# NCAR/SPERR

Measured on AMD Instinct MI355X. Metric: compress+decompress GB/s/GPU on 256^3 fp32 chunks @ BPP=2.0; bitstream-exact vs ref, higher is better.
Workload: dtype f64; 1 GPU; synthetic 1024^3 fp32 turbulence per GPU, 256^3 chunks, BPP=2.0, step = compress + decompress, volume and container resident in HBM; chunks_per_gpu=64, parallelism=chunks farmed over 1 GPU(s), no collective

## Files before the change

sperr_amd/csrc/engine.hip:

```cpp
#include <algorithm>
#include <array>
#include <chrono>
#include <cstdlib>
#include <cstring>
#include <atomic>
#include <deque>
#include <map>
#include <memory>
#include <condition_variable>
#include <mutex>
#include <numeric>
#include <thread>
#include <string>
#include <vector>

#include "../../include/sperr_hip.h"
#include "engine_internal.h"
#include "host_container.hpp"
#include "speck_dec.h"
#include "dequant.h"
#include "speck_enc.h"
#include "speck_tree_host.hpp"
#include "outlier.h"
#include "quality.h"
// ... 365 lines not shown
    return false;
  return lift2_applicable(P.fwd[3].region);
}
constexpr uint32_t kLevel2Floor = 96;
static bool plan_level2(const ShapePlan& P)
{
  const char* env = getenv("SPERR_HIP_XYZ_LEVEL2");
  const int sw = env ? atoi(env) : 1;
  if (sw == 0 || !level2_fits(P))
    return false;
  const uint32_t* r = P.fwd[3].region;
  return sw == 2 || std::min(r[0], std::min(r[1], r[2])) >= kLevel2Floor;
}

static void plan_schedule(ShapePlan& P)
{
  LiftSchedule& S = P.schedule;
  S = LiftSchedule{};
  S.pass.resize(P.fwd.size());
  for (size_t k = 0; k < P.fwd.size(); k++)
    S.pass[k].fuse = pass_fuse_rule(P, k, S.pass[k].inner);
  S.head = fuse_xyz(P) ? LiftSchedule::kHeadXYZ : fuse_xy(P) ? LiftSchedule::kHeadXY : LiftSchedule::kNoHead;
  S.fusable = plan_fusable(P);
  S.brick = S.head == LiftSchedule::kHeadXYZ && S.fusable && P.fwd.size() >= 3;
  for (size_t k = 3; k < P.fwd.size(); k++)
    for (int a = 0; a < 3; a++)
      S.coarseBox[a] = std::max(S.coarseBox[a], P.fwd[k].region[a]);
  S.level2 = plan_level2(P);
}

constexpr int kHiMaxK = 9;
static bool use_lis_hi(const ShapePlan& P, bool tables)
{
  static const bool hiEnv = !(getenv("SPERR_HIP_LIS_HI") && atoi(getenv("SPERR_HIP_LIS_HI")) == 0);
  return hiEnv && tables && P.ht.grids.size() <= 288 && P.ht.roots.size() <= 48 &&
         P.maxK >= 1 && P.maxK <= kHiMaxK;
}
static bool use_tables(const ShapePlan& P)
{
  if (!P.ht.allRegular || P.maxK < 1)
    return false;
  return use_lis_hi(P, true);
}
static bool use_mixed(const ShapePlan& P, bool tables)
{
  static const bool mixEnv = !(getenv("SPERR_HIP_LIS_MIXED") && atoi(getenv("SPERR_HIP_LIS_MIXED")) == 0);
  const bool twoD = (P.ht.flags & spk::kTree2D) != 0;
  if ((!twoD && !mixEnv) || tables || P.ht.cls.empty() || P.ht.roots.size() > 48 || P.ht.grids.size() > 352 ||
      P.ht.mxSlot.size() != P.ht.cls.size())
    return false;
  return 2 * kMxS + 256 <= kMxRing && ((kMxS + kMxM) >> 6) + 5 <= 64 && kMxM >= 192 &&
         mx_smem_bytes(kMxS, kMxM, kMxQ) <= 138u * 1024u;
}
static DecPlanHost plan_list_kernels(const ShapePlan& P, bool tables)
{
  DecPlanHost ph{P.d_initLIS, P.d_initLen, tables, P.l0Level >= 0 && P.ht.grids.size() <= 288,
                 P.l1Level >= 0 && P.ht.grids.size() <= 288, P.maxK};
  ph.l2 = ph.l1 && P.l2Level >= 0;
  ph.hi = use_lis_hi(P, ph.tables);
  ph.mixed = use_mixed(P, tables);
  return ph;
}

int build_plan(ShapePlan& P, size_t dx, size_t dy, size_t dz, bool twoD = false)
{
  const unsigned __int128 samples = (unsigned __int128)dx * dy * dz;
  if (dx == 0 || dy == 0 || dz == 0 || dx > 0xffff || dy > 0xffff || dz > 0xffff || samples > (1ull << 31)) {
    fprintf(stderr, "[sperr_hip] chunk of %zu x %zu x %zu not supported (at most 65535 per axis, 2^31 samples)\n",
            dx, dy, dz);
    return -1;
  }
  P.dims[0] = (uint32_t)dx;
  P.dims[1] = (uint32_t)dy;
  P.dims[2] = (uint32_t)dz;
  P.N = (uint32_t)(dx * dy * dz);
  P.ht = spk::build_tree(dx, dy, dz, twoD, false);
  P.maxK = 0;
  for (const auto& lc : P.ht.levelClass)
    P.maxK = std::max<int>(P.maxK, lc.K);
  const bool tables = use_tables(P);
  if (!tables)
    spk::build_mx_columns(P.ht);
  const spk::HostTree& h = P.ht;
  const uint32_t nlev = h.nlevels;

  std::vector<uint32_t> cap(nlev), levelOff(nlev + 1, 0), initLen(nlev);
  for (uint32_t l = 0; l < nlev; l++) {
    cap[l] = std::max<uint32_t>(h.levelCap[l], (uint32_t)h.initLIS[l].size());
    levelOff[l + 1] = levelOff[l] + cap[l];
    initLen[l] = (uint32_t)h.initLIS[l].size();
  }
  P.lisEntries = levelOff[nlev] + 8;
  std::vector<uint64_t> initLIS(levelOff[nlev] ? levelOff[nlev] : 1, 0);
  for (uint32_t l = 0; l < nlev; l++)
    for (size_t k = 0; k < h.initLIS[l].size(); k++)
      initLIS[levelOff[l] + k] = h.initLIS[l][k];

  std::vector<uint16_t> tileLevel;
  std::vector<uint32_t> tileStart, levelFirstTile(nlev, 0), levelNumTiles(nlev, 0);
  for (uint32_t l = nlev; l-- > 0;) {
    levelFirstTile[l] = (uint32_t)tileLevel.size();
    const uint32_t nt = (cap[l] + kListTile - 1) / kListTile;
    levelNumTiles[l] = nt;
    for (uint32_t t = 0; t < nt; t++) {
      tileLevel.push_back((uint16_t)l);
      tileStart.push_back(t * kListTile);
    }
  }
  P.nListTiles = (uint32_t)tileLevel.size();

  std::vector<uint32_t> depthBlocks;
  P.depthBlockOff.assign(h.maxDepth + 1, 0);
  for (uint32_t d = 0; d < h.maxDepth; d++) {
// ... 4533 lines not shown
```

sperr_amd/csrc/speck_dec.h:

```cpp
#ifndef SPERR_AMD_SPECK_DEC_H
#define SPERR_AMD_SPECK_DEC_H

#include "common.h"

namespace sperrhip {

struct DecState {
  uint32_t active;
  int32_t done;
  uint32_t error;
  int32_t nbp;
  uint32_t cur;
  uint32_t nLip, nRef;
  uint32_t nLeafEv;
  int32_t lastPlane;
  int32_t refPlaneP1;
  uint32_t refPartial;
  uint64_t pos;
  uint64_t avail;
  uint64_t total_bits;
  uint64_t payload;
  uint64_t lipStart, lipBits;
  uint32_t l0Ticket;
  int32_t l0PlaneP1;
// ... 90 lines not shown
  uint32_t queueCap;
  size_t queueStride;
  uint64_t* sigbits;
  size_t sigbitsStride;
  uint32_t treeTabLen;
  uint64_t* leafEv;
  uint32_t leafCap;
  size_t leafStride;
  uint16_t* leafState;
  size_t leafStateStride;
  uint8_t* leafDirty;
  size_t leafDirtyStride;
  const uint32_t* wordLeaf;
  unsigned long long* l0Flags;
  size_t l0FlagStride;
  int32_t l0Level;
  unsigned long long* l0Tab;
  unsigned long long* l1Flags;
  int32_t l1Level;
  unsigned long long* l2Flags;
  int32_t l2Level;
  uint64_t* lisStamps;
  unsigned long long* hiFlags;
  size_t hiFlagStride;
  uint32_t hiW;
  uint32_t hiK;
  uint32_t hiSmemBytes;
  uint32_t hiHop2;
  uint32_t hiGroupsMax;
  uint32_t hiExtra;
  uint32_t hiCand;
  uint32_t hiAhead;
  const uint64_t* iRoots;
  uint32_t iLevels;
  const uint8_t* mxSlot;
  const uint8_t* mxLevelGroup;
  uint32_t mxS, mxM;
  uint32_t mxQ;
  uint32_t mxSmemBytes;
};

struct DecPlanHost {
  const uint64_t* d_initLIS;
  const uint32_t* d_initLen;
  bool tables;
  bool l0;
  bool l1;
  int maxK;
  bool hi = false;
  bool l2 = false;
  bool mixed = false;
  uint32_t gridDiv = 1;
  uint32_t mxGroups = 0;
  bool skipFinish = false;
  uint32_t* d_live = nullptr;
  uint32_t* h_live = nullptr;
  hipEvent_t* liveEv = nullptr;
};
constexpr int kLiveSlots = 24;

constexpr int kTabWMax = 28672;
__host__ __device__ inline uint32_t tab_window(int K, uint32_t smemBytes)
{
  const uint32_t perBit8 = 8u * (uint32_t)(2 * (2 * K - 1) + 4) + 1u;
  const uint32_t fixed = 4 * 8 + 130 * 4 + (uint32_t)(2 * K) * 8 + 64;
  uint32_t w = (uint32_t)(((uint64_t)(smemBytes - fixed) * 8) / perBit8);
  w = w / 1024 * 1024;
  if (w > (uint32_t)kTabWMax)
    w = kTabWMax;
  return w;
}

__host__ __device__ inline uint32_t hi_window(int K, uint32_t smemBytes, uint32_t hop2 = 1)
{
  const uint32_t perBit8 = 8u * (uint32_t)(2 * (2 * K - 1) + (hop2 ? 8 : 4)) + 1u;
  const uint32_t fixed = 4 * 8 + 2 * 130 * 4 + (uint32_t)(2 * K) * 8 + 64;
  uint32_t w = (uint32_t)(((uint64_t)(smemBytes - fixed) * 8) / perBit8);
  w = w / 256 * 256;
  if (w > (uint32_t)kTabWMax)
    w = kTabWMax;
  return w;
}

constexpr int kMxWordsPerRegion = 8;
constexpr uint32_t kMxS = 2048, kMxM = 768, kMxQ = 1024, kMxRing = 8192;
uint32_t mx_smem_bytes(uint32_t S, uint32_t M, uint32_t Q);
int prepare_lis_mx(const DecBuffers& b);
int launch_lis_mx(hipStream_t stream, const DecBuffers& b, int p, uint32_t groups, bool stamps);

int launch_speck_decode(hipStream_t stream, const DecBuffers& b, const DecPlanHost& plan,
                        const uint8_t* container, const uint64_t* d_chunkOff,
                        const uint64_t* d_chunkLen, bool wide_pass, int maxPlanes);

}
#endif
```

sperr_amd/csrc/speck_dec.hip:

```cpp
#include "speck_dec.h"
#include "dequant.h"
#include "bit_words.h"
#include "lis_chain.h"

namespace sperrhip {

using namespace spk;

#define DEC_ACTIVE_OR_RETURN(s, p)                               \
  if (!(s).active || (s).done || (int)(p) >= (s).nbp)            \
    return;

__device__ __forceinline__ uint64_t get64(const uint64_t* words, uint64_t pos)
{
  const uint64_t lo = words[pos >> 6];
  const int sh = (int)(pos & 63);
  return sh ? (lo >> sh) | (words[(pos >> 6) + 1] << (64 - sh)) : lo;
}

__global__ void k_dec_header(DecBuffers b, const uint8_t* container, const uint64_t* chunkOff,
                             const uint64_t* chunkLen, const uint64_t* initLIS,
                             const uint32_t* initLen, int wide_pass)
{
  const uint32_t c = blockIdx.x * blockDim.x + threadIdx.x;
// ... 27 lines not shown
      s.error = 1;
    return;
  }
  cs.mean = d1;
  cs.q = d2;
  if (len < 17 + 9) {
    s.error = 1;
    return;
  }
  const int nbp = p[17];
  uint64_t total_bits;
  memcpy(&total_bits, p + 18, 8);
  uint64_t avail = (len - 26) * 8;
  if (avail > total_bits)
    avail = total_bits;
  s.nbp = nbp;
  s.avail = avail;
  s.total_bits = total_bits;
  s.payload = chunkOff[c] + 26;
  cs.wide = nbp > 32 ? 1u : 0u;
  cs.nbp = nbp;
  cs.total_bits = total_bits;
  s.active = (nbp > 0 && (int)cs.wide == wide_pass) ? 1u : 0u;
  s.iPart = b.iLevels;
  for (uint32_t l = 0; l < b.tree.nlevels; l++) {
    s.listLen[0][l] = initLen[l];
    s.listLen[1][l] = 0;
    for (uint32_t k = 0; k < initLen[l]; k++)
      b.lis[0][c * b.lisStride + b.levelOff[l] + k] = initLIS[b.levelOff[l] + k];
  }
}

__global__ void __launch_bounds__(kThreads)
k_dec_load_words(DecBuffers b, const uint8_t* container)
{
  const uint32_t c = blockIdx.y;
  const DecState& s = b.st[c];
  if (!s.active)
    return;
  const uint64_t nbytes = (s.avail + 7) / 8;
  const uint64_t w = (uint64_t)blockIdx.x * blockDim.x + threadIdx.x;
  if (w * 8 >= nbytes)
    return;
  const uint8_t* p = container + s.payload + w * 8;
  uint64_t v = 0;
  const int n = (int)min((uint64_t)8, nbytes - w * 8);
  for (int k = 0; k < n; k++)
    v |= (uint64_t)p[k] << (8 * k);
  b.stream[c * b.streamStride + w] = v;
}

constexpr int kDecTileWords = kThreads;

__device__ __forceinline__ bool leaf_word(const DecBuffers& b, uint32_t c, uint32_t wi,
                                          uint64_t& born, uint64_t& sig, uint64_t& neg, uint32_t tag)
{
  born = sig = neg = 0;
  if (b.wordLeaf == nullptr)
    return false;
  const uint32_t wl = b.wordLeaf[wi];
  if (wl == 0xffffffffu)
    return false;
  if (tag && b.leafDirty[c * b.leafDirtyStride + (wl >> 5)] != (uint8_t)tag)
    return false;
  const uint32_t sel = (wl & 3u) * 2u;
  const uint4* q = reinterpret_cast<const uint4*>(b.leafState + c * b.leafStateStride + (wl & ~31u));
  uint32_t v[16];
  uint32_t any = 0;
#pragma unroll
  for (int k = 0; k < 4; k++) {
    const uint4 t = q[k];
    v[4 * k] = t.x;
    v[4 * k + 1] = t.y;
    v[4 * k + 2] = t.z;
    v[4 * k + 3] = t.w;
    any |= t.x | t.y | t.z | t.w;
  }
  if (!any)
    return false;
  uint32_t bo[2] = {0, 0}, si[2] = {0, 0}, ne[2] = {0, 0};
#pragma unroll
  for (int k = 0; k < 16; k++) {
    const int h = k >> 3, sh = (k & 7) * 4;
    const uint32_t a = v[k] & 0xffffu, d = v[k] >> 16;
    const uint32_t s4 = ((a >> sel) & 3u) | (((d >> sel) & 3u) << 2);
    const uint32_t n4 = ((a >> (8 + sel)) & 3u) | (((d >> (8 + sel)) & 3u) << 2);
    const uint32_t b4 = ((a & 0xffu) ? 3u : 0u) | ((d & 0xffu) ? 12u : 0u);
    si[h] |= s4 << sh;
    ne[h] |= n4 << sh;
    bo[h] |= b4 << sh;
  }
  born = (uint64_t)bo[0] | ((uint64_t)bo[1] << 32);
  sig = (uint64_t)si[0] | ((uint64_t)si[1] << 32);
  neg = (uint64_t)ne[0] | ((uint64_t)ne[1] << 32);
  return true;
}

__global__ void __launch_bounds__(kThreads) k_dec_count(DecBuffers b, int p)
{
  const uint32_t c = blockIdx.y;
  const DecState& s = b.st[c];
  DEC_ACTIVE_OR_RETURN(s, p);
  __shared__ uint32_t sm[kThreads / 64 + 1];
  __shared__ uint32_t sh_need;
  const uint32_t nw = (b.tree.nvals + 63) / 64;
  constexpr uint32_t kAhead = 8;
  for (uint32_t tile0 = blockIdx.x; tile0 < b.nPixTiles; tile0 += gridDim.x * kAhead) {
  uint32_t needMask = 0;
  const bool skipTest = b.tileBorn != nullptr && b.wordLeaf != nullptr;
  if (skipTest) {
    if (threadIdx.x == 0)
      sh_need = 0;
    uint32_t wl[kAhead], tb[kAhead];
#pragma unroll
    for (uint32_t q = 0; q < kAhead; q++) {
      const uint32_t tile = tile0 + q * gridDim.x;
      const uint32_t wi = tile * kDecTileWords + threadIdx.x;
      tb[q] = tile < b.nPixTiles ? (uint32_t)b.tileBorn[c * b.tileStride + tile] : 0u;
      wl[q] = (tile < b.nPixTiles && wi < nw) ? b.wordLeaf[wi] : 0xfffffffeu;
    }
    uint32_t mine = 0;
#pragma unroll
    for (uint32_t q = 0; q < kAhead; q++) {
      const uint32_t tile = tile0 + q * gridDim.x;
      if (tile >= b.nPixTiles)
        continue;
      bool need = tb[q] != 0;
      if (!need && wl[q] != 0xfffffffeu)
        need = wl[q] == 0xffffffffu || b.leafDirty[c * b.leafDirtyStride + (wl[q] >> 5)] == (uint8_t)(p + 2);
      mine |= need ? 1u << q : 0u;
    }
    __syncthreads();
    if (mine)
      atomicOr(&sh_need, mine);
    __syncthreads();
    needMask = sh_need;
  }
  for (uint32_t q = 0; q < kAhead; q++) {
  const uint32_t tile = tile0 + q * gridDim.x;
  if (tile >= b.nPixTiles)
    break;
  const uint32_t wi = tile * kDecTileWords + threadIdx.x;
  if (skipTest && !((needMask >> q) & 1u)) {
    if (threadIdx.x == 0) {
      b.tileLip[c * b.tileStride + tile] = 0;
      b.tileRef[c * b.tileStride + tile] = 0;
    }
    continue;
// ... 11 lines not shown
      if (lb & ~born) {
        born |= lb;
        b.bornM[c * b.maskPixStride + wi] = born;
      }
      if (ln) {
        const uint64_t sg = b.sign[c * b.signStride + wi];
        if (sg & ln)
          b.sign[c * b.signStride + wi] = sg & ~ln;
      }
    }
    if (fresh | (ls & ~sig)) {
      if (b.refPlanes) {
        const uint64_t found = (fresh | ls) & ~sig;
        if (found && (uint32_t)(p + 1) < b.refNPlanes) {
          uint64_t* pw = b.refPlanes + c * b.refPlaneStride + ref_plane_word((uint32_t)(p + 1), wi);
          *pw = sig ? (*pw | found) : found;
          if (!sig)
            b.wordTop[c * b.wordTopStride + wi] = (uint8_t)(p + 2);
        }
      }
      sig |= fresh | ls;
      *so = sig;
    }
    if (fresh)
      *sn = 0;
    const uint64_t lip = born & ~sig;
    v = (uint32_t)__popcll(lip) | ((uint32_t)__popcll(sig) << 16);
    anyBorn = born != 0;
  }
  if (b.tileBorn != nullptr) {
    const int anyB = __syncthreads_or(anyBorn ? 1 : 0);
    if (threadIdx.x == 0 && anyB)
      b.tileBorn[c * b.tileStride + tile] = 1;
  }
  uint32_t r = v;
#pragma unroll
  for (int d = 32; d > 0; d >>= 1)
    r += (uint32_t)__shfl_xor((int)r, d, 64);
  __syncthreads();
  if ((threadIdx.x & 63) == 0)
    sm[threadIdx.x >> 6] = r;
  __syncthreads();
  if (threadIdx.x == 0) {
    uint32_t tot = 0;
    for (int w = 0; w < kThreads / 64; w++)
      tot += sm[w];
    b.tileLip[c * b.tileStride + tile] = tot & 0xffffu;
    b.tileRef[c * b.tileStride + tile] = tot >> 16;
  }
  }
  }
}

__global__ void __launch_bounds__(kThreads) k_dec_scan(DecBuffers b, int p)
{
  const uint32_t c = blockIdx.x;
  DecState& s = b.st[c];
  DEC_ACTIVE_OR_RETURN(s, p);
  __shared__ uint64_t sm[kThreads / 64 + 1];
  uint32_t* tl = b.tileLip + c * b.tileStride;
  uint32_t* tr = b.tileRef + c * b.tileStride;
  uint32_t* ol = b.tileLipOff + c * b.tileStride;
  uint32_t* orr = b.tileRefOff + c * b.tileStride;
  uint64_t carry = 0;
  for (uint32_t base = 0; base < b.nPixTiles; base += kThreads) {
    const uint32_t i = base + threadIdx.x;
    const uint64_t v = i < b.nPixTiles ? ((uint64_t)tl[i] | ((uint64_t)tr[i] << 32)) : 0;
    uint64_t total;
    const uint64_t ex = block_exclusive_scan<uint64_t>(v, sm, &total) + carry;
    if (i < b.nPixTiles) {
      ol[i] = (uint32_t)ex;
      orr[i] = (uint32_t)(ex >> 32);
    }
    carry += total;
  }
  if (threadIdx.x == 0) {
    s.nLip = (uint32_t)carry;
    s.nRef = (uint32_t)(carry >> 32);
    s.lipStart = s.pos;
    s.l0Ticket = 0;
    s.l1Ticket = 0;
    s.l2Ticket = 0;
    s.hiTicket = 0;
    s.hiCompactDone = 0;
    s.bornCount = 0;
    s.leafCount = 0;
    for (int g = 0; g < 8; g++)
      s.hiBornCnt[g] = s.hiLeafCnt[g] = 0;
  }
}

__global__ void __launch_bounds__(kThreads) k_lip_deposit(DecBuffers b, int p)
{
  const uint32_t c = blockIdx.y;
  const DecState& s = b.st[c];
  DEC_ACTIVE_OR_RETURN(s, p);
  if (s.nLip == 0)
    return;
  __shared__ uint32_t sm[kThreads / 64 + 1];
  const uint32_t nw = (b.tree.nvals + 63) / 64;
  const uint64_t* rs = b.lipSig + c * b.lipResStride;
  const uint64_t* rn = b.lipNeg + c * b.lipResStride;
  for (uint32_t tile = blockIdx.x; tile < b.nPixTiles; tile += gridDim.x) {
    if (b.tileLip[c * b.tileStride + tile] == 0)
      continue;
    const uint32_t wi = tile * kDecTileWords + threadIdx.x;
    uint64_t lip = 0;
    if (wi < nw)
      lip = b.bornM[c * b.maskPixStride + wi] & ~b.sigOld[c * b.maskPixStride + wi];
    uint32_t total;
    const uint32_t ex = block_exclusive_scan<uint32_t>((uint32_t)__popcll(lip), sm, &total) +
                        b.tileLipOff[c * b.tileStride + tile];
    const uint32_t n = (uint32_t)__popcll(lip);
    if (n == 0)
      continue;
    const uint32_t sh = ex & 63u;
    uint64_t vs = rs[ex >> 6] >> sh, vn = rn[ex >> 6] >> sh;
    if (sh && sh + n > 64) {
      vs |= rs[(ex >> 6) + 1] << (64 - sh);
      vn |= rn[(ex >> 6) + 1] << (64 - sh);
    }
    if (n < 64) {
      vs &= (1ull << n) - 1;
      vn &= (1ull << n) - 1;
    }
    if (vs == 0)
      continue;
    uint64_t outS = vs, outN = vn;
    spread_under_mask(lip, outS, outN);
    b.sigNew[c * b.maskPixStride + wi] |= outS;
    if (outN)
      b.sign[c * b.signStride + wi] &= ~outN;
  }
}

__device__ __forceinline__ uint64_t lip_word(const uint64_t* words, const DecState& s,
                                             uint64_t w, uint64_t nbits)
{
  const uint64_t pos = s.lipStart + w * 64;
  uint64_t v = get64(words, pos);
  if (pos + 64 > s.avail)
    v = pos >= s.avail ? 0 : (v & ((1ull << (s.avail - pos)) - 1));
// ... 2755 lines not shown
        CT v2 = cv[u];
        if (v2 == 0)
          v2 = initPrev;
        if (p >= 1)
          v2 = sw[u] ? v2 + half : v2 - half;
        else if (sw[u])
          v2 += 1;
        coef[idx[u]] = v2;
      }
    }
    LDS_ONLY_BARRIER();
  }
}

__global__ void __launch_bounds__(kThreads) k_ref_deposit(DecBuffers b, int p)
{
  const uint32_t c = blockIdx.y;
  const DecState& s = b.st[c];
  DEC_ACTIVE_OR_RETURN(s, p);
  if ((uint32_t)p >= b.refNPlanes)
    return;
  __shared__ uint32_t sm[kThreads / 64 + 1];
  const uint32_t nw = (b.tree.nvals + 63) / 64;
  const uint64_t* words = b.stream + c * b.streamStride;
  uint64_t* planes = b.refPlanes + c * b.refPlaneStride;
  const uint64_t avail = s.avail, pos0 = s.pos;
  const bool partial = pos0 + (uint64_t)s.nRef > avail;
  for (uint32_t tile = blockIdx.x; tile < b.nPixTiles; tile += gridDim.x) {
    if (b.tileRef[c * b.tileStride + tile] == 0)
      continue;
    const uint32_t wi = tile * kDecTileWords + threadIdx.x;
    const uint64_t sig = wi < nw ? b.sigOld[c * b.maskPixStride + wi] : 0ull;
    const uint32_t cnt = (uint32_t)__popcll(sig);
    uint32_t total;
    const uint32_t o = block_exclusive_scan_lds<uint32_t>(cnt, sm, &total);
    if (cnt == 0)
      continue;
    const uint64_t at = pos0 + (uint64_t)b.tileRefOff[c * b.tileStride + tile] + o;
    const uint32_t n = at >= avail ? 0u : (uint32_t)min((uint64_t)cnt, avail - at);
    uint64_t res = 0, got = 0;
    if (n) {
      const uint64_t bits = get64(words, at);
      res = n < 64 ? bits & ((1ull << n) - 1) : bits;
      got = n < 64 ? (1ull << n) - 1 : ~0ull;
      if (cnt != 64)
        spread_under_mask(sig, res, got);
    }
    planes[ref_plane_word((uint32_t)p, wi)] = res;
    if (partial)
      b.refMask[c * b.maskPixStride + wi] = got;
  }
}

__global__ void __launch_bounds__(kThreads) k_ref_assemble(DecBuffers b)
{
  const uint32_t c = blockIdx.y;
  const DecState& s = b.st[c];
  const uint32_t nw = (uint32_t)(b.coefStride / 64);
  const uint32_t nwv = (b.tree.nvals + 63) / 64;
  const uint32_t lane = threadIdx.x & 63u;
  uint32_t* coef = reinterpret_cast<uint32_t*>(b.coef) + c * b.coefStride;
  constexpr uint32_t kW = 8;
  const uint32_t wave = (uint32_t)__builtin_amdgcn_readfirstlane((int)((blockIdx.x * kThreads + threadIdx.x) >> 6));
  const uint32_t nwave = (gridDim.x * kThreads) >> 6;
  if (!s.active || s.nbp == 0) {
    for (uint32_t w = wave; w < nw; w += nwave)
      coef[(size_t)w * 64 + lane] = 0;
    return;
  }
  const int lastPlane = s.lastPlane, refPlane = s.refPlaneP1 - 1;
  const bool partial = s.refPartial != 0;
  const int pLow = refPlane >= 0 ? refPlane : lastPlane + 1;
  const int nbp = min(s.nbp, (int)b.refNPlanes);
  const uint64_t* planes = b.refPlanes + c * b.refPlaneStride;
  const uint64_t* sigOld = b.sigOld + c * b.maskPixStride;
  const uint64_t* sigNew = b.sigNew + c * b.maskPixStride;
  const uint64_t* refMask = b.refMask + c * b.maskPixStride;
  const uint8_t* wordTop = b.wordTop + c * b.wordTopStride;
  const int scheme = b.coefSigned != 0 ? coef_scheme(s) : 0;
  const uint64_t* sign = b.sign + c * b.signStride;
  for (uint32_t w0 = wave * kW; w0 + kW <= nw; w0 += nwave * kW) {
    uint64_t so[kW], sn[kW], rm[kW], sg[kW];
    int top[kW], maxTop = 0;
    uint64_t any = 0;
    const uint32_t tops[2] = {reinterpret_cast<const uint32_t*>(wordTop + w0)[0], reinterpret_cast<const uint32_t*>(wordTop + w0)[1]};
#pragma unroll
    for (uint32_t u = 0; u < kW; u++) {
      const uint32_t w = w0 + u;
      const bool in = w < nwv;
      so[u] = sigOld[w];
      sn[u] = sigNew[w];
      rm[u] = refMask[w];
      sg[u] = sign[in ? w : 0u];
      if (!in)
        so[u] = sn[u] = 0;
      top[u] = so[u] ? min((int)((tops[u >> 2] >> (8 * (u & 3))) & 0xffu), nbp) : 0;
      maxTop = max(maxTop, top[u]);
      any |= so[u] | sn[u];
    }
    uint32_t M[kW];
#pragma unroll
    for (uint32_t u = 0; u < kW; u++)
      M[u] = 0;
    if (any && maxTop > pLow) {
      const int nPl = maxTop - pLow;
      const uint32_t myU = lane & 7u, myPs = lane >> 3;
// ... 55 lines not shown
        if (scheme)
          v = coef_scheme_pack(v, ((sg[u] >> lane) & 1ull) != 0, scheme);
      }
      coef[(size_t)w * 64 + lane] = v;
    }
  }
}

__global__ void __launch_bounds__(kThreads) k_dec_fold(DecBuffers b)
{
  const uint32_t c = blockIdx.y;
  const DecState& s = b.st[c];
  if (!s.active || s.nbp == 0)
    return;
  const uint32_t nw = (b.tree.nvals + 63) / 64;
  const uint32_t wi = blockIdx.x * blockDim.x + threadIdx.x;
  if (wi >= nw)
    return;
  uint64_t lb, ls, ln;
  if (!leaf_word(b, c, wi, lb, ls, ln, (uint32_t)s.lastPlane + 1u))
    return;
  const uint64_t fresh = ls & ~b.sigOld[c * b.maskPixStride + wi];
  if (fresh)
    b.sigNew[c * b.maskPixStride + wi] |= fresh;
  if (ln) {
    const uint64_t sg = b.sign[c * b.signStride + wi];
    if (sg & ln)
      b.sign[c * b.signStride + wi] = sg & ~ln;
  }
}

template <typename CT>
__global__ void __launch_bounds__(kThreads) k_dec_finish(DecBuffers b)
{
  const uint32_t c = blockIdx.y;
  const DecState& s = b.st[c];
  if (!s.active || s.nbp == 0)
    return;
  const uint32_t n = b.tree.nvals;
  const uint32_t i = blockIdx.x * blockDim.x + threadIdx.x;
  if (i >= n)
    return;
  const uint64_t m = 1ull << (i & 63);
  const bool isNew = (b.sigNew[c * b.maskPixStride + (i >> 6)] & m) != 0;
  const bool isOld = (b.sigOld[c * b.maskPixStride + (i >> 6)] & m) != 0;
  if (!isNew && !isOld)
    return;
  CT* coef = reinterpret_cast<CT*>(b.coef) + c * b.coefStride;
  if (coef[i] != 0)
    return;
  coef[i] = never_refined<CT>(s.lastPlane + (isNew ? 0 : 1));
}

__global__ void k_dec_plane_end(DecBuffers b, int p)
{
  const uint32_t c = blockIdx.x * blockDim.x + threadIdx.x;
  if (c >= b.nchunks)
    return;
  DecState& s = b.st[c];
  DEC_ACTIVE_OR_RETURN(s, p);
  const uint64_t room = s.avail - s.pos;
  s.refPlaneP1 = p + 1;
  s.refPartial = (uint64_t)s.nRef > room ? 1u : 0u;
  s.pos += min((uint64_t)s.nRef, room);
  if (s.pos >= s.avail || p == 0)
    s.done = 1;
}

__global__ void __launch_bounds__(kThreads) k_dec_live(DecBuffers b, uint32_t* out)
{
  uint32_t live = 0;
  for (uint32_t c = threadIdx.x; c < b.nchunks; c += blockDim.x)
    live += (b.st[c].active && !b.st[c].done) ? 1u : 0u;
  live = (uint32_t)__syncthreads_count(live != 0);
  if (threadIdx.x == 0)
    *out = live;
}

int launch_speck_decode(hipStream_t stream, const DecBuffers& b, const DecPlanHost& plan,
                        const uint8_t* container, const uint64_t* d_chunkOff,
                        const uint64_t* d_chunkLen, bool wide_pass, int maxPlanes)
{
  const uint32_t nc = b.nchunks;
  const dim3 perChunk((nc + 63) / 64);
  LAUNCH_K(k_dec_header, perChunk, dim3(64), 0, stream, b, container, d_chunkOff,
                     d_chunkLen, plan.d_initLIS, plan.d_initLen, wide_pass ? 1 : 0);
  const uint32_t wordBlocks = (uint32_t)((b.streamStride + kThreads - 1) / kThreads);
  LAUNCH_K(k_dec_load_words, dim3(wordBlocks, nc), dim3(kThreads), 0, stream, b,
                     container);
  const uint32_t tokBlocks = (uint32_t)((b.tokStride + kThreads - 1) / kThreads);
  const uint32_t gdiv = std::max<uint32_t>(1u, plan.gridDiv);
  static const uint32_t tileCapEnv = tune_getenv("SPERR_HIP_TILE_GRID") ? (uint32_t)atoi(tune_getenv("SPERR_HIP_TILE_GRID")) : 0u;
  const uint32_t tileCap = tileCapEnv ? tileCapEnv : 1536u;
  const uint32_t tokSegGrid = capped_blocks((uint32_t)(b.tokStride / kLipSeg + 1), nc, kGridCap / gdiv);
  const uint32_t tokGrid = capped_blocks(tokBlocks, nc, kGridCap / gdiv), tileGrid = capped_blocks(b.nPixTiles, nc, tileCap / gdiv);
  static const uint32_t l0Total = tune_getenv("SPERR_HIP_L0_WGS") ? (uint32_t)atoi(tune_getenv("SPERR_HIP_L0_WGS")) : 512u;
  static const uint32_t l01Cap = tune_getenv("SPERR_HIP_L01_CAP") ? (uint32_t)atoi(tune_getenv("SPERR_HIP_L01_CAP")) : 64u;
  const uint32_t l0Groups = std::min<uint32_t>(l01Cap, std::max<uint32_t>(1, l0Total / nc));
  if (plan.tables && plan.l0) {
    if (set_max_dyn_lds(reinterpret_cast<const void*>(&k_lis_l0), (int)kL0Smem) ||
        set_max_dyn_lds(reinterpret_cast<const void*>(&k_lis_l1), (int)kL1Smem) ||
        set_max_dyn_lds(reinterpret_cast<const void*>(&k_lis_l2), (int)kL2Smem))
      return -1;
  }
  static const uint32_t l1Total = tune_getenv("SPERR_HIP_L1_WGS") ? (uint32_t)atoi(tune_getenv("SPERR_HIP_L1_WGS")) : 512u;
  const uint32_t l1Groups = std::min<uint32_t>(l01Cap, std::max<uint32_t>(1, l1Total / nc));
  static const uint32_t l2Total = tune_getenv("SPERR_HIP_L2_WGS") ? (uint32_t)atoi(tune_getenv("SPERR_HIP_L2_WGS")) : 512u;
  const uint32_t l2Groups = std::min<uint32_t>(l01Cap, std::max<uint32_t>(1, l2Total / nc));
  static const uint32_t l2Min = tune_getenv("SPERR_HIP_L2_MIN") ? (uint32_t)std::max(1, atoi(tune_getenv("SPERR_HIP_L2_MIN"))) : 512u;
  const uint32_t placeGrid = capped_blocks((uint32_t)((b.bornStride + kThreads - 1) / kThreads), nc, kGridCap / gdiv);
  static const uint32_t hiTotal = tune_getenv("SPERR_HIP_HI_WGS") ? (uint32_t)atoi(tune_getenv("SPERR_HIP_HI_WGS")) : 128u;
  const uint32_t hiGroups = std::min<uint32_t>(std::max<uint32_t>(1, b.hiGroupsMax), std::max<uint32_t>(1, hiTotal / nc));
  static const uint32_t mxTotal = getenv("SPERR_HIP_MX_WGS") ? (uint32_t)atoi(getenv("SPERR_HIP_MX_WGS")) : 208u;
  const uint32_t mxGroups = std::min<uint32_t>(std::min<uint32_t>(8u, std::max<uint32_t>(1, b.hiGroupsMax)),
                                               plan.mxGroups ? plan.mxGroups : std::max<uint32_t>(1, mxTotal / nc));
  if (plan.mixed && prepare_lis_mx(b))
    return -1;
  if (plan.tables && plan.hi) {
    if (set_max_dyn_lds(reinterpret_cast<const void*>(&k_lis_hi<uint32_t>), (int)b.hiSmemBytes) ||
        set_max_dyn_lds(reinterpret_cast<const void*>(&k_lis_hi<uint64_t>), (int)b.hiSmemBytes))
      return -1;
  }
#define LAUNCH_CT(kern, ...)                    \
  do {                                          \
    if constexpr (sizeof(CT) == 4)              \
      LAUNCH_K(kern<uint32_t>, __VA_ARGS__);    \
    else                                        \
      LAUNCH_K(kern<uint64_t>, __VA_ARGS__);    \
  } while (0)
  auto plane = [&](auto ct, int p) -> int {
    using CT = decltype(ct);
    LAUNCH_K(k_dec_count, dim3(tileGrid, nc), dim3(kThreads), 0, stream, b, p);
    LAUNCH_K(k_dec_scan, dim3(nc), dim3(kThreads), 0, stream, b, p);
    LAUNCH_K(k_lip_words, dim3(tokSegGrid, nc), dim3(kThreads), 0, stream, b, p);
    LAUNCH_K(k_lip_scan, dim3(nc), dim3(kThreads), 0, stream, b, p);
    LAUNCH_CT(k_lip_apply, dim3(tokGrid, nc), dim3(kThreads), 0, stream, b, p);
    LAUNCH_K(k_lip_deposit, dim3(tileGrid, nc), dim3(kThreads), 0, stream, b, p);
    if (plan.tables) {
      if (plan.l0)
        LAUNCH_K(k_lis_l0, dim3(l0Groups, nc), dim3(kL0Threads), kL0Smem, stream, b, p);
      if (plan.l1)
        LAUNCH_K(k_lis_l1, dim3(l1Groups, nc), dim3(kL1Threads), kL1Smem, stream, b, p);
      if (plan.l2)
        LAUNCH_K(k_lis_l2, dim3(l2Groups, nc), dim3(kL2Threads), kL2Smem, stream, b, p, l2Min);
      if (!plan.hi)
        return -1;
      LAUNCH_CT(k_lis_hi, dim3(hiGroups, nc), dim3(kTabThreads), b.hiSmemBytes, stream, b, p);
      LAUNCH_K(k_lis_compact, dim3(b.tree.nlevels, nc), dim3(kTabThreads), 0, stream, b, p);
    }
    else if (plan.mixed) {
      if (launch_lis_mx(stream, b, p, mxGroups, b.lisStamps != nullptr))
        return -1;
      LAUNCH_K(k_lis_compact, dim3(b.tree.nlevels, nc), dim3(kTabThreads), 0, stream, b, p);
    }
    else
      LAUNCH_CT(k_lis_walk, dim3(nc), dim3(64), 0, stream, b, p);
    if (plan.tables || plan.mixed) {
      if (b.nSlots) {
        LAUNCH_K(k_place_scan, dim3(b.nSlots, nc), dim3(kTabThreads), 0, stream, b, p);
        LAUNCH_K(k_place_scatter, dim3(placeGrid, nc), dim3(kThreads), 0, stream, b, p);
      }
      LAUNCH_K(k_leaf_apply, dim3(capped_blocks(1024, nc, kGridCap / gdiv), nc), dim3(kThreads), 0, stream, b, p);
    }
    if (b.refPlanes && sizeof(CT) == 4)
      LAUNCH_K(k_ref_deposit, dim3(tileGrid, nc), dim3(kThreads), 0, stream, b, p);
    else
      LAUNCH_CT(k_ref_apply2, dim3(tileGrid, nc), dim3(kThreads), 0, stream, b, p);
    return 0;
  };
#undef LAUNCH_CT
  for (int p = maxPlanes - 1; p >= 0; p--) {
    if (wide_pass ? plane(uint64_t{}, p) : plane(uint32_t{}, p))
      return -1;
    LAUNCH_K(k_dec_plane_end, perChunk, dim3(64), 0, stream, b, p);
    const int planesDone = maxPlanes - p;
    if (plan.d_live && p > 0 && planesDone >= 16 && planesDone % 2 == 0 && plan.h_live && plan.liveEv) {
      const int k = (planesDone - 16) / 2;
      if (k < kLiveSlots) {
        LAUNCH_K(k_dec_live, dim3(1), dim3(kThreads), 0, stream, b, plan.d_live + k);
        HIP_CHECK(hipMemcpyAsync(plan.h_live + k, plan.d_live + k, sizeof(uint32_t), hipMemcpyDeviceToHost, stream));
        HIP_CHECK(hipEventRecord(plan.liveEv[k], stream));
        if (k >= 1) {
          HIP_CHECK(hipEventSynchronize(plan.liveEv[k - 1]));
          if (plan.h_live[k - 1] == 0)
            break;
        }
      }
    }
  }
  {
    const uint32_t n = b.tree.nvals;
    if ((plan.tables || plan.mixed) && b.wordLeaf)
      LAUNCH_K(k_dec_fold, dim3(((n + 63) / 64 + kThreads - 1) / kThreads, nc), dim3(kThreads), 0,
               stream, b);
    if (b.refPlanes && !wide_pass)
      LAUNCH_K(k_ref_assemble, dim3(capped_blocks((uint32_t)((b.coefStride / 64 + 15) / 16), nc, kGridCapWide), nc),
               dim3(kThreads), 0, stream, b);
    if (!plan.skipFinish) {
      if (wide_pass)
        LAUNCH_K(k_dec_finish<uint64_t>, dim3((n + kThreads - 1) / kThreads, nc), dim3(kThreads), 0,
                 stream, b);
      else
        LAUNCH_K(k_dec_finish<uint32_t>, dim3((n + kThreads - 1) / kThreads, nc), dim3(kThreads), 0,
                 stream, b);
    }
  }
  HIP_CHECK(hipGetLastError());
  return 0;
}

}
```

Measured before the change: 69.84 GB/s.

## Fuse refinement deposit with next plane's pixel count and scan into turn kernels

Adds a k_pix_turn kernel that does the current plane's refinement-bit deposit and the next plane's per-tile count pass in one sweep over the pixel tiles. It prefetches the next word's state and skips tiles that need no work. A k_dec_turn kernel then merges the plane-end bookkeeping with the next plane's scan. Together these replace four kernel launches per bit plane with two, and cut repeated reads of the sig, born and leaf state. The fused path is on by default for large chunks and can be disabled with SPERR_HIP_PIX_TURN=0. It adds complexity to bitstream-exact ordering and register pressure from the prefetch.

```diff
diff --git a/sperr_amd/csrc/engine.hip b/sperr_amd/csrc/engine.hip
--- a/sperr_amd/csrc/engine.hip
+++ b/sperr_amd/csrc/engine.hip
@@ -441,6 +441,17 @@
   return 2 * kMxS + 256 <= kMxRing && ((kMxS + kMxM) >> 6) + 5 <= 64 && kMxM >= 192 &&
          mx_smem_bytes(kMxS, kMxM, kMxQ) <= 138u * 1024u;
 }
+constexpr uint32_t kPixTurnFloor = 64;
+static bool plan_pix_turn(const ShapePlan& P)
+{
+  const char* env = getenv("SPERR_HIP_PIX_TURN");
+  const int sw = env ? atoi(env) : 1;
+  if (sw == 0)
+    return false;
+  const size_t decTiles = (round_up((size_t)P.N, 512) / 64 + kThreads - 1) / kThreads;
+  return sw == 2 || decTiles >= kPixTurnFloor;
+}
+
 static DecPlanHost plan_list_kernels(const ShapePlan& P, bool tables)
 {
   DecPlanHost ph{P.d_initLIS, P.d_initLen, tables, P.l0Level >= 0 && P.ht.grids.size() <= 288,
@@ -448,6 +459,7 @@
   ph.l2 = ph.l1 && P.l2Level >= 0;
   ph.hi = use_lis_hi(P, ph.tables);
   ph.mixed = use_mixed(P, tables);
+  ph.pixTurn = plan_pix_turn(P);
   return ph;
 }
 
diff --git a/sperr_amd/csrc/speck_dec.h b/sperr_amd/csrc/speck_dec.h
--- a/sperr_amd/csrc/speck_dec.h
+++ b/sperr_amd/csrc/speck_dec.h
@@ -166,6 +166,7 @@
   bool mixed = false;
   uint32_t gridDiv = 1;
   uint32_t mxGroups = 0;
+  bool pixTurn = false;
   bool skipFinish = false;
   uint32_t* d_live = nullptr;
   uint32_t* h_live = nullptr;
diff --git a/sperr_amd/csrc/speck_dec.hip b/sperr_amd/csrc/speck_dec.hip
--- a/sperr_amd/csrc/speck_dec.hip
+++ b/sperr_amd/csrc/speck_dec.hip
@@ -103,6 +103,42 @@
 
 constexpr int kDecTileWords = kThreads;
 
+__device__ __forceinline__ bool leaf_states(const DecBuffers& b, uint32_t c, uint32_t wl,
+                                            uint64_t& born, uint64_t& sig, uint64_t& neg)
+{
+  const uint32_t sel = (wl & 3u) * 2u;
+  const uint4* q = reinterpret_cast<const uint4*>(b.leafState + c * b.leafStateStride + (wl & ~31u));
+  uint32_t v[16];
+  uint32_t any = 0;
+#pragma unroll
+  for (int k = 0; k < 4; k++) {
+    const uint4 t = q[k];
+    v[4 * k] = t.x;
+    v[4 * k + 1] = t.y;
+    v[4 * k + 2] = t.z;
+    v[4 * k + 3] = t.w;
+    any |= t.x | t.y | t.z | t.w;
+  }
+  if (!any)
+    return false;
+  uint32_t bo[2] = {0, 0}, si[2] = {0, 0}, ne[2] = {0, 0};
+#pragma unroll
+  for (int k = 0; k < 16; k++) {
+    const int h = k >> 3, sh = (k & 7) * 4;
+    const uint32_t a = v[k] & 0xffffu, d = v[k] >> 16;
+    const uint32_t s4 = ((a >> sel) & 3u) | (((d >> sel) & 3u) << 2);
+    const uint32_t n4 = ((a >> (8 + sel)) & 3u) | (((d >> (8 + sel)) & 3u) << 2);
+    const uint32_t b4 = ((a & 0xffu) ? 3u : 0u) | ((d & 0xffu) ? 12u : 0u);
+    si[h] |= s4 << sh;
+    ne[h] |= n4 << sh;
+    bo[h] |= b4 << sh;
+  }
+  born = (uint64_t)bo[0] | ((uint64_t)bo[1] << 32);
+  sig = (uint64_t)si[0] | ((uint64_t)si[1] << 32);
+  neg = (uint64_t)ne[0] | ((uint64_t)ne[1] << 32);
+  return true;
+}
+
 __device__ __forceinline__ bool leaf_word(const DecBuffers& b, uint32_t c, uint32_t wi,
                                           uint64_t& born, uint64_t& sig, uint64_t& neg, uint32_t tag)
 {
@@ -114,37 +150,7 @@
     return false;
   if (tag && b.leafDirty[c * b.leafDirtyStride + (wl >> 5)] != (uint8_t)tag)
     return false;
-  const uint32_t sel = (wl & 3u) * 2u;
-  const uint4* q = reinterpret_cast<const uint4*>(b.leafState + c * b.leafStateStride + (wl & ~31u));
-  uint32_t v[16];
-  uint32_t any = 0;
-#pragma unroll
-  for (int k = 0; k < 4; k++) {
-    const uint4 t = q[k];
-    v[4 * k] = t.x;
-    v[4 * k + 1] = t.y;
-    v[4 * k + 2] = t.z;
-    v[4 * k + 3] = t.w;
-    any |= t.x | t.y | t.z | t.w;
-  }
-  if (!any)
-    return false;
-  uint32_t bo[2] = {0, 0}, si[2] = {0, 0}, ne[2] = {0, 0};
-#pragma unroll
-  for (int k = 0; k < 16; k++) {
-    const int h = k >> 3, sh = (k & 7) * 4;
-    const uint32_t a = v[k] & 0xffffu, d = v[k] >> 16;
-    const uint32_t s4 = ((a >> sel) & 3u) | (((d >> sel) & 3u) << 2);
-    const uint32_t n4 = ((a >> (8 + sel)) & 3u) | (((d >> (8 + sel)) & 3u) << 2);
-    const uint32_t b4 = ((a & 0xffu) ? 3u : 0u) | ((d & 0xffu) ? 12u : 0u);
-    si[h] |= s4 << sh;
-    ne[h] |= n4 << sh;
-    bo[h] |= b4 << sh;
-  }
-  born = (uint64_t)bo[0] | ((uint64_t)bo[1] << 32);
-  sig = (uint64_t)si[0] | ((uint64_t)si[1] << 32);
-  neg = (uint64_t)ne[0] | ((uint64_t)ne[1] << 32);
-  return true;
+  return leaf_states(b, c, wl, born, sig, neg);
 }
 
 __global__ void __launch_bounds__(kThreads) k_dec_count(DecBuffers b, int p)
@@ -262,12 +268,8 @@
   }
 }
 
-__global__ void __launch_bounds__(kThreads) k_dec_scan(DecBuffers b, int p)
+__device__ __forceinline__ void dec_scan_chunk(const DecBuffers& b, DecState& s, uint32_t c, uint64_t* sm)
 {
-  const uint32_t c = blockIdx.x;
-  DecState& s = b.st[c];
-  DEC_ACTIVE_OR_RETURN(s, p);
-  __shared__ uint64_t sm[kThreads / 64 + 1];
   uint32_t* tl = b.tileLip + c * b.tileStride;
   uint32_t* tr = b.tileRef + c * b.tileStride;
   uint32_t* ol = b.tileLipOff + c * b.tileStride;
@@ -298,6 +300,15 @@
     for (int g = 0; g < 8; g++)
       s.hiBornCnt[g] = s.hiLeafCnt[g] = 0;
   }
+}
+
+__global__ void __launch_bounds__(kThreads) k_dec_scan(DecBuffers b, int p)
+{
+  const uint32_t c = blockIdx.x;
+  DecState& s = b.st[c];
+  DEC_ACTIVE_OR_RETURN(s, p);
+  __shared__ uint64_t sm[kThreads / 64 + 1];
+  dec_scan_chunk(b, s, c, sm);
 }
 
 __global__ void __launch_bounds__(kThreads) k_lip_deposit(DecBuffers b, int p)
@@ -3159,6 +3170,233 @@
   }
 }
 
+struct PixWord {
+  uint64_t sig, fresh, born;
+  uint32_t wl;
+  uint32_t refOff;
+};
+__device__ __forceinline__ PixWord pix_word_load(const DecBuffers& b, uint32_t c, uint32_t tile0, uint32_t todo,
+                                                 uint32_t refTiles, uint32_t countTiles, uint32_t nw)
+{
+  PixWord w{0ull, 0ull, 0ull, 0xffffffffu, 0u};
+  if (todo == 0)
+    return w;
+  const uint32_t q = (uint32_t)__ffs((int)todo) - 1u;
+  const uint32_t tile = tile0 + q * gridDim.x;
+  const uint32_t wi = tile * kDecTileWords + threadIdx.x;
+  if ((refTiles >> q) & 1u)
+    w.refOff = b.tileRefOff[c * b.tileStride + tile];
+  if (wi < nw) {
+    w.sig = b.sigOld[c * b.maskPixStride + wi];
+    if ((countTiles >> q) & 1u) {
+      w.fresh = b.sigNew[c * b.maskPixStride + wi];
+      w.born = b.bornM[c * b.maskPixStride + wi];
+      if (b.wordLeaf != nullptr)
+        w.wl = b.wordLeaf[wi];
+    }
+  }
+  return w;
+}
+
+__global__ void __launch_bounds__(kThreads, 5) k_pix_turn(DecBuffers b, int p)
+{
+  const uint32_t c = blockIdx.y;
+  const DecState& s = b.st[c];
+  if (!s.active || s.done)
+    return;
+  const bool inPlane = p < s.nbp;
+  const uint64_t avail = s.avail, pos0 = s.pos;
+  const uint32_t nRef = s.nRef;
+  const bool refOn = inPlane && (uint32_t)p < b.refNPlanes;
+  const bool endsHere = inPlane && (p == 0 || (uint64_t)nRef >= avail - pos0);
+  const bool countOn = !endsHere && p - 1 >= 0 && p - 1 < s.nbp;
+  if (!refOn && !countOn)
+    return;
+  const bool partial = inPlane && pos0 + (uint64_t)nRef > avail;
+  __shared__ uint32_t smRef[2][kThreads / 64];
+  __shared__ uint32_t smCnt[2][kThreads / 64];
+  __shared__ uint32_t smBorn[2][kThreads / 64];
+  uint32_t refRow = 0, cntRow = 0;
+  __shared__ uint32_t sh_need[2];
+  const uint32_t nw = (b.tree.nvals + 63) / 64;
+  const uint64_t* words = b.stream + c * b.streamStride;
+  constexpr uint32_t kAhead = 8;
+  const bool skipTest = b.tileBorn != nullptr && b.wordLeaf != nullptr;
+  uint32_t round = 0;
+  for (uint32_t tile0 = blockIdx.x; tile0 < b.nPixTiles; tile0 += gridDim.x * kAhead, round ^= 1u) {
+    uint32_t needMask = 0, refMaskT = 0;
+    if (refOn) {
+#pragma unroll
+      for (uint32_t q = 0; q < kAhead; q++) {
+        const uint32_t tile = tile0 + q * gridDim.x;
+        if (tile < b.nPixTiles && b.tileRef[c * b.tileStride + tile] != 0)
+          refMaskT |= 1u << q;
+      }
+    }
+    if (countOn && skipTest) {
+      if (threadIdx.x == 0)
+        sh_need[round] = 0;
+      uint32_t wl[kAhead], tb[kAhead];
+#pragma unroll
+      for (uint32_t q = 0; q < kAhead; q++) {
+        const uint32_t tile = tile0 + q * gridDim.x;
+        const uint32_t wi = tile * kDecTileWords + threadIdx.x;
+        tb[q] = tile < b.nPixTiles ? (uint32_t)b.tileBorn[c * b.tileStride + tile] : 0u;
+        wl[q] = (tile < b.nPixTiles && wi < nw) ? b.wordLeaf[wi] : 0xfffffffeu;
+      }
+      uint32_t mine = 0;
+#pragma unroll
+      for (uint32_t q = 0; q < kAhead; q++) {
+        const uint32_t tile = tile0 + q * gridDim.x;
+        if (tile >= b.nPixTiles)
+          continue;
+        bool need = tb[q] != 0;
+        if (!need && wl[q] != 0xfffffffeu)
+          need = wl[q] == 0xffffffffu || b.leafDirty[c * b.leafDirtyStride + (wl[q] >> 5)] == (uint8_t)(p + 1);
+        mine |= need ? 1u << q : 0u;
+      }
+      __syncthreads();
+      if (mine)
+        atomicOr(&sh_need[round], mine);
+      __syncthreads();
+      needMask = sh_need[round];
+    }
+    else if (countOn)
+      needMask = (1u << kAhead) - 1u;
+    uint32_t todo = 0;
+    for (uint32_t q = 0; q < kAhead; q++) {
+      const uint32_t tile = tile0 + q * gridDim.x;
+      if (tile >= b.nPixTiles)
+        break;
+      if (countOn && !((needMask >> q) & 1u) && threadIdx.x == 0) {
+        b.tileLip[c * b.tileStride + tile] = 0;
+        b.tileRef[c * b.tileStride + tile] = 0;
+      }
+      todo |= (((refMaskT | needMask) >> q) & 1u) << q;
+    }
+    PixWord nx = pix_word_load(b, c, tile0, todo, refMaskT, needMask, nw);
+    uint32_t nxDirty = 0;
+    if (nx.wl != 0xffffffffu)
+      nxDirty = b.leafDirty[c * b.leafDirtyStride + (nx.wl >> 5)];
+    while (todo) {
+      const uint32_t q = (uint32_t)__ffs((int)todo) - 1u;
+      todo &= todo - 1u;
+      const uint32_t tile = tile0 + q * gridDim.x;
+      const uint32_t wi = tile * kDecTileWords + threadIdx.x;
+      const bool doRef = (refMaskT >> q) & 1u, doCount = (needMask >> q) & 1u;
+      const bool in = wi < nw;
+      const PixWord cur = nx;
+      const uint32_t curDirty = nxDirty;
+      nx = pix_word_load(b, c, tile0, todo, refMaskT, needMask, nw);
+      uint64_t sig = cur.sig;
+      uint32_t cnt = 0, n = 0;
+      uint64_t at = 0;
+      if (doRef) {
+        cnt = (uint32_t)__popcll(sig);
+        const uint32_t inc = wave_inclusive_scan(cnt);
+        if ((threadIdx.x & 63u) == 63u)
+          smRef[refRow][threadIdx.x >> 6] = inc;
+        LDS_ONLY_BARRIER();
+        uint32_t base = 0;
+        for (uint32_t w = 0; w < (threadIdx.x >> 6); w++)
+          base += smRef[refRow][w];
+        refRow ^= 1u;
+        at = pos0 + (uint64_t)cur.refOff + base + inc - cnt;
+        n = (cnt == 0 || at >= avail) ? 0u : (uint32_t)min((uint64_t)cnt, avail - at);
+      }
+      const bool hasRef = cnt != 0;
+      uint64_t w0 = 0, w1 = 0;
+      if (n) {
+        w0 = words[at >> 6];
+        w1 = words[(at >> 6) + 1];
+      }
+      if (nx.wl != 0xffffffffu)
+        nxDirty = b.leafDirty[c * b.leafDirtyStride + (nx.wl >> 5)];
+      uint64_t lb = 0, ls = 0, ln = 0;
+      bool leafHit = false;
+      if (cur.wl != 0xffffffffu && curDirty == (uint32_t)(uint8_t)(p + 1) && cur.born != ~0ull)
+        leafHit = leaf_states(b, c, cur.wl, lb, ls, ln);
+      uint64_t res = 0, got = 0;
+      if (n) {
+        const int sh = (int)(at & 63);
+        const uint64_t bits = sh ? (w0 >> sh) | (w1 << (64 - sh)) : w0;
+        res = n < 64 ? bits & ((1ull << n) - 1) : bits;
+        got = n < 64 ? (1ull << n) - 1 : ~0ull;
+        if (cnt != 64)
+          spread_under_mask(sig, res, got);
+      }
+      uint64_t* pw = b.refPlanes + c * b.refPlaneStride + ref_plane_word((uint32_t)p, wi);
+      if (!doCount) {
+        if (hasRef) {
+          *pw = res;
+          if (partial)
+            b.refMask[c * b.maskPixStride + wi] = got;
+        }
+        continue;
+      }
+      uint32_t v = 0;
+      bool anyBorn = false;
+      if (in) {
+        const uint64_t fresh = cur.fresh;
+        uint64_t born = cur.born;
+        if (leafHit) {
+          if (lb & ~born) {
+            born |= lb;
+            b.bornM[c * b.maskPixStride + wi] = born;
+          }
+          if (ln) {
+            const uint64_t sg = b.sign[c * b.signStride + wi];
+            if (sg & ln)
+              b.sign[c * b.signStride + wi] = sg & ~ln;
+          }
+        }
+        uint64_t found = 0;
+        if (fresh | (ls & ~sig)) {
+          found = (fresh | ls) & ~sig;
+          if ((uint32_t)p >= b.refNPlanes)
+            found = 0;
+        }
+        if (hasRef || found) {
+          *pw = res | found;
+          if (!sig)
+            b.wordTop[c * b.wordTopStride + wi] = (uint8_t)(p + 1);
+        }
+        if (fresh | (ls & ~sig)) {
+          sig |= fresh | ls;
+          b.sigOld[c * b.maskPixStride + wi] = sig;
+        }
+        if (fresh)
+          b.sigNew[c * b.maskPixStride + wi] = 0;
+        const uint64_t lip = born & ~sig;
+        v = (uint32_t)__popcll(lip) | ((uint32_t)__popcll(sig) << 16);
+        anyBorn = born != 0;
+      }
+      uint32_t r = v;
+#pragma unroll
+      for (int d = 32; d > 0; d >>= 1)
+        r += (uint32_t)__shfl_xor((int)r, d, 64);
+      const bool waveBorn = __ballot(anyBorn ? 1 : 0) != 0ull;
+      if ((threadIdx.x & 63u) == 0u) {
+        smCnt[cntRow][threadIdx.x >> 6] = r;
+        smBorn[cntRow][threadIdx.x >> 6] = waveBorn ? 1u : 0u;
+      }
+      LDS_ONLY_BARRIER();
+      if (threadIdx.x == 0) {
+        uint32_t tot = 0, anyB = 0;
+        for (int w = 0; w < kThreads / 64; w++) {
+          tot += smCnt[cntRow][w];
+          anyB |= smBorn[cntRow][w];
+        }
+        b.tileLip[c * b.tileStride + tile] = tot & 0xffffu;
+        b.tileRef[c * b.tileStride + tile] = tot >> 16;
+        if (b.tileBorn != nullptr && anyB)
+          b.tileBorn[c * b.tileStride + tile] = 1;
+      }
+      cntRow ^= 1u;
+    }
+  }
+}
+
 __global__ void __launch_bounds__(kThreads) k_ref_assemble(DecBuffers b)
 {
   const uint32_t c = blockIdx.y;
@@ -3320,6 +3558,16 @@
   coef[i] = never_refined<CT>(s.lastPlane + (isNew ? 0 : 1));
 }
 
+__device__ __forceinline__ void dec_plane_end_chunk(DecState& s, int p)
+{
+  const uint64_t room = s.avail - s.pos;
+  s.refPlaneP1 = p + 1;
+  s.refPartial = (uint64_t)s.nRef > room ? 1u : 0u;
+  s.pos += min((uint64_t)s.nRef, room);
+  if (s.pos >= s.avail || p == 0)
+    s.done = 1;
+}
+
 __global__ void k_dec_plane_end(DecBuffers b, int p)
 {
   const uint32_t c = blockIdx.x * blockDim.x + threadIdx.x;
@@ -3327,12 +3575,28 @@
     return;
   DecState& s = b.st[c];
   DEC_ACTIVE_OR_RETURN(s, p);
-  const uint64_t room = s.avail - s.pos;
-  s.refPlaneP1 = p + 1;
-  s.refPartial = (uint64_t)s.nRef > room ? 1u : 0u;
-  s.pos += min((uint64_t)s.nRef, room);
-  if (s.pos >= s.avail || p == 0)
-    s.done = 1;
+  dec_plane_end_chunk(s, p);
+}
+
+__global__ void __launch_bounds__(kThreads) k_dec_turn(DecBuffers b, int pEnd, int pBegin)
+{
+  const uint32_t c = blockIdx.x;
+  DecState& s = b.st[c];
+  __shared__ uint64_t sm[kThreads / 64 + 1];
+  __shared__ int sh_on;
+  if (threadIdx.x == 0) {
+    int on = 0;
+    if (s.active && !s.done) {
+      if (pEnd < s.nbp)
+        dec_plane_end_chunk(s, pEnd);
+      on = (!s.done && pBegin >= 0 && pBegin < s.nbp) ? 1 : 0;
+    }
+    sh_on = on;
+  }
+  LDS_ONLY_BARRIER();
+  if (!sh_on)
+    return;
+  dec_scan_chunk(b, s, c, sm);
 }
 
 __global__ void __launch_bounds__(kThreads) k_dec_live(DecBuffers b, uint32_t* out)
@@ -3396,10 +3660,17 @@
     else                                        \
       LAUNCH_K(kern<uint64_t>, __VA_ARGS__);    \
   } while (0)
+  const bool pixTurn = plan.pixTurn && b.refPlanes != nullptr && !wide_pass;
+  auto turn = [&](int p) {
+    LAUNCH_K(k_pix_turn, dim3(tileGrid, nc), dim3(kThreads), 0, stream, b, p);
+    LAUNCH_K(k_dec_turn, dim3(nc), dim3(kThreads), 0, stream, b, p, p - 1);
+  };
   auto plane = [&](auto ct, int p) -> int {
     using CT = decltype(ct);
-    LAUNCH_K(k_dec_count, dim3(tileGrid, nc), dim3(kThreads), 0, stream, b, p);
-    LAUNCH_K(k_dec_scan, dim3(nc), dim3(kThreads), 0, stream, b, p);
+    if (!pixTurn) {
+      LAUNCH_K(k_dec_count, dim3(tileGrid, nc), dim3(kThreads), 0, stream, b, p);
+      LAUNCH_K(k_dec_scan, dim3(nc), dim3(kThreads), 0, stream, b, p);
+    }
     LAUNCH_K(k_lip_words, dim3(tokSegGrid, nc), dim3(kThreads), 0, stream, b, p);
     LAUNCH_K(k_lip_scan, dim3(nc), dim3(kThreads), 0, stream, b, p);
     LAUNCH_CT(k_lip_apply, dim3(tokGrid, nc), dim3(kThreads), 0, stream, b, p);
@@ -3430,17 +3701,23 @@
       }
       LAUNCH_K(k_leaf_apply, dim3(capped_blocks(1024, nc, kGridCap / gdiv), nc), dim3(kThreads), 0, stream, b, p);
     }
-    if (b.refPlanes && sizeof(CT) == 4)
-      LAUNCH_K(k_ref_deposit, dim3(tileGrid, nc), dim3(kThreads), 0, stream, b, p);
-    else
-      LAUNCH_CT(k_ref_apply2, dim3(tileGrid, nc), dim3(kThreads), 0, stream, b, p);
+    if (pixTurn)
+      turn(p);
+    else {
+      if (b.refPlanes && sizeof(CT) == 4)
+        LAUNCH_K(k_ref_deposit, dim3(tileGrid, nc), dim3(kThreads), 0, stream, b, p);
+      else
+        LAUNCH_CT(k_ref_apply2, dim3(tileGrid, nc), dim3(kThreads), 0, stream, b, p);
+      LAUNCH_K(k_dec_plane_end, perChunk, dim3(64), 0, stream, b, p);
+    }
     return 0;
   };
 #undef LAUNCH_CT
+  if (pixTurn && maxPlanes > 0)
+    turn(maxPlanes);
   for (int p = maxPlanes - 1; p >= 0; p--) {
     if (wide_pass ? plane(uint64_t{}, p) : plane(uint32_t{}, p))
       return -1;
-    LAUNCH_K(k_dec_plane_end, perChunk, dim3(64), 0, stream, b, p);
     const int planesDone = maxPlanes - p;
     if (plan.d_live && p > 0 && planesDone >= 16 && planesDone % 2 == 0 && plan.h_live && plan.liveEv) {
       const int k = (planesDone - 16) / 2;
```

After: 70.64 GB/s, median of 6. 1.01x the previous value.
